# donahowe/TheaterGen

Hardware: AMD Instinct MI355X
Metric: 512px 50-step char images/sec (node), CMIGBench 4-turn story (higher is better)
Workload: dtype bf16; 1 GPU; SD-1.5 512x512, 4-turn story x 2 characters = 8 char images per step per GPU, 50 DDIM steps, CFG 7.5, IP-Adapter 77+4 tokens scale 0.4, bf16, random-init weights; plan=sd15, char_batch=8, cfg_batch=16, streams=1, ddim_steps=50, parallelism=dialogue-sharded x1 (RCCL broadcast + all_gather only)

## Files before the change

include/theatergen_hip.h:

```cpp
#ifndef THEATERGEN_HIP_H
#define THEATERGEN_HIP_H

#include <stdint.h>

#ifdef __cplusplus
extern "C" {
#endif

#define TG_BF16 0
#define TG_F16 1

#define TG_OK 0
#define TG_ERR_ARG (-1)
#define TG_ERR_LAUNCH (-2)
#define TG_ERR_UNSUPPORTED (-3)

#define TG_ACT_NONE 0
#define TG_ACT_SILU 1
#define TG_ACT_GELU 2
#define TG_ACT_QUICK_GELU 3

#define TG_ABI_VERSION 308
int tg_version(void);
const char* tg_last_error(void);
// ... 217 lines not shown
  int32_t dtype;
  const void* x; int64_t ldx;
  const void* wpk;
  const void* res; int64_t ldres;
  void* out; int64_t ldc;
  int64_t M;
  int32_t N, K;
  int32_t ln;
  float ln_eps;
  int32_t variant;
  const float* v640;
  const float* u640;
} tg_rc_linear_desc;
int tg_rc_linear(const tg_rc_linear_desc* d, void* stream);
int tg_rc_linear_dup(const tg_rc_linear_desc* d, int64_t c_dup_offset, void* stream);

typedef struct {
  int32_t dtype;
  const void* h; int64_t ldh;
  const void* wq;
  const void* kv;
  const void* wo;
  void* out; int64_t ldc;
  int64_t M;
  int32_t rows_per_batch;
  int32_t text_len, ip_tokens;
  float ln_eps;
  const float* ip_scale;
} tg_rc_xattn_desc;
int tg_rc_xattn(const tg_rc_xattn_desc* d, void* stream);
int tg_rc_kv_pack(int32_t dtype, int32_t batch, const void* k, const void* vt, int64_t ldt, int32_t text_len, const void* kip,
                  const void* vtip, int64_t ldi, int32_t ip_tokens, void* out, void* stream);

typedef struct {
  int32_t dtype;
  const void* h; int64_t ldh;
  const void* w1;
  const void* w2;
  const float* b2;
  const void* wpo;
  const void* res0; int64_t ldres;
  void* out; int64_t ldc;
  int64_t M;
  int32_t inner;
  float ln_eps;
  int32_t dbg;
} tg_rc_ff_desc;
int tg_rc_ff(const tg_rc_ff_desc* d, void* stream);

typedef struct {
  int32_t dtype;
  const void* x; int64_t ldx;
  const float* coef;
  const void* win;
  const void* wqkv;
  void* y; int64_t ldy;
  void* qk; int64_t ldqk;
  void* vt; int64_t ldt;
  int64_t M;
  int32_t rows_per_batch;
  float ln_eps;
  int32_t dbg;
} tg_rc_front_desc;
int tg_rc_front(const tg_rc_front_desc* d, void* stream);

typedef struct {
// ... 50 lines not shown
```

theatergen_amd/_lib.py:

```python
import ctypes as C
import os

HERE = os.path.dirname(os.path.abspath(__file__))
LIB_PATH = os.environ.get("THEATERGEN_HIP_LIB") or os.path.join(HERE, "lib", "libtheatergen_hip.so")

TG_BF16, TG_F16 = 0, 1
ABI_VERSION = 308
ACT_NONE, ACT_SILU, ACT_GELU, ACT_QUICK_GELU = 0, 1, 2, 3

i32, i64, f32, vp = C.c_int32, C.c_int64, C.c_float, C.c_void_p


class GemmDesc(C.Structure):
    _fields_ = [
        ("dtype", i32), ("mode", i32), ("a0", vp), ("a1", vp), ("c0", i32), ("c1", i32),
        ("batch", i32), ("in_h", i32), ("in_w", i32), ("out_h", i32), ("out_w", i32),
        ("stride", i32), ("upsample", i32), ("w", vp), ("M", i64), ("N", i64), ("K", i64),
        ("bias", vp), ("bvec", vp), ("ldbvec", i64), ("rows_per_batch", i64), ("res", vp), ("ldres", i64),
        ("act", i32), ("geglu", i32), ("out_scale", f32), ("out", vp), ("ldc", i64), ("n_split", i64),
        ("out_t", vp), ("ldt", i64), ("workspace", vp), ("workspace_bytes", i64),
        ("force_split_k", i32), ("force_tile", i32), ("a_rows_per_batch", i64), ("a_batch_stride", i64),
        ("pad_mode", i32), ("a_silu", i32), ("a_coef", vp), ("ln_u", vp), ("ln_v", vp), ("ln_eps", f32), ("ln_rows", vp),
        ("lda", i64), ("ldw", i64), ("out_gn_partials", vp), ("out_gn_groups", i32),
    ]


class AttnDesc(C.Structure):
    _fields_ = [
        ("dtype", i32), ("batch", i32), ("heads", i32), ("head_dim", i32), ("n_q", i32),
        ("q", vp), ("q_ld", i64), ("q_bs", i64),
        ("k0", vp), ("k0_ld", i64), ("k0_bs", i64), ("vt0", vp), ("vt0_ld", i64), ("vt0_bs", i64), ("len0", i32),
        ("k1", vp), ("k1_ld", i64), ("k1_bs", i64), ("vt1", vp), ("vt1_ld", i64), ("vt1_bs", i64), ("len1", i32),
        ("scale", f32), ("w1", f32), ("out", vp), ("out_ld", i64), ("out_bs", i64), ("causal", i32), ("w1_dev", vp),
        ("mask", vp), ("mask_bs", i64), ("mask_hs", i64), ("mask_qs", i64),
    ]


class AttnBwdDesc(C.Structure):
    _fields_ = [
        ("dtype", i32), ("batch", i32), ("heads", i32), ("head_dim", i32), ("n", i32),
        ("q", vp), ("k", vp), ("v", vp), ("dout", vp), ("ld", i64), ("bs", i64),
# ... 191 lines not shown
```

theatergen_amd/build.py:

```python
import hashlib
import os
import subprocess
import sys
from concurrent.futures import ThreadPoolExecutor

HERE = os.path.dirname(os.path.abspath(__file__))
CSRC = os.path.join(HERE, "csrc")
OBJ = os.path.join(CSRC, "_build")
LIBDIR = os.path.join(HERE, "lib")
LIB = os.path.join(LIBDIR, "libtheatergen_hip.so")
HEADER = os.path.join(os.path.dirname(HERE), "include", "theatergen_hip.h")
ARCH = "gfx950"
FLAGS = ["--offload-arch=" + ARCH, "-O3", "-std=c++17", "-fPIC",
         "-Wno-unused-result"]


EXTRA_FLAGS = {"tg_rowchain.hip": ["-mllvm", "-pragma-unroll-threshold=1000000"]}

BUILD_INFO = os.path.join(LIBDIR, "build_info.json")


def _write_build_info():
    import json

# ... 58 lines not shown
            f.write(r.stderr)
        with open(stamp, "w") as f:
            f.write(dg)

    if todo:
        with ThreadPoolExecutor(max_workers=min(8, len(todo))) as ex:
            list(ex.map(compile_one, todo))
    if todo or not os.path.exists(LIB):
        cmd = [hipcc, "--offload-arch=" + ARCH, "-shared", "-fPIC", "-o", LIB] + objs
        if verbose:
            print("[build]", " ".join(cmd), flush=True)
        r = subprocess.run(cmd, capture_output=True, text=True)
        if r.returncode != 0:
            raise RuntimeError(f"link failed:\n{r.stdout}\n{r.stderr}")
    if todo or not os.path.exists(BUILD_INFO):
        _write_build_info()
    if check_gate or os.environ.get("TG_BUILD_GATE") == "1":
        write_resources(check=True, verbose=verbose, report=False)
    return LIB


RESOURCES_JSON = os.path.join(os.path.dirname(HERE), "profiles", "r6_kernel_resources.json")
HOT_GATES = [
    ("attention_kernel<bf16,48,64,true,true,false,false>", 0, 128),
    ("attention_kernel<f16,48,64,true,true,false,false>", 0, 128),
    ("attention_kernel<", 0, 256),
    ("attention_wide_kernel<", 0, 256),
    ("gemm_glds_kernel<", 0, 256),
    ("conv_halo_kernel<", 0, 256),
    ("conv_slab_kernel<", 320, 256),
    ("bt_gemm_kernel<", 132, 256),
    ("rc_xattn_kernel<", 0, 256),
    ("rc_ff_kernel<", 0, 256),
    ("rc_front_kernel<", 0, 216),
    ("rc_linear_kernel<", 0, 256),
    ("skinny_gemm_kernel<", 0, 256),
    ("attn_bwd_kernel<4,2,", 0, 224),
    ("attn_bwd_kernel<", 0, 256),
    ("pp_gemm_kernel<bf16,2,", 0, 256),
    ("pp_gemm_kernel<f16,2,", 0, 256),
    ("pp_gemm_kernel<bf16,0,0>", 0, 256),
    ("pp_gemm_kernel<f16,0,0>", 0, 256),
    ("pp_gemm_kernel<", 256, 256),
    ("conv_in_mfma_kernel<", 0, 256),
    ("conv_out_mfma_kernel<", 0, 128),
    ("step_epilogue_kernel<", 0, 40),
]


def _pretty(sym):
    import re
    m = re.match(r"_ZN12_GLOBAL__N_1(\d+)", sym) or re.match(r"_Z(\d+)", sym)
    if not m:
        return sym
    n = int(m.group(1))
    base, rest = sym[m.end():m.end() + n], sym[m.end() + n:]
    if not rest.startswith("I"):
        return base
    args, i = [], 1
    while i < len(rest) and rest[i] != "E":
        if rest.startswith("DF16b", i):
            args.append("bf16"); i += 5
        elif rest.startswith("DF16_", i):
            args.append("f16"); i += 5
        elif rest.startswith("NS_", i):
            m = re.match(r"NS_(\d+)", rest[i:])
# ... 160 lines not shown
```

theatergen_amd/csrc/tg_rowchain.hip:

```cpp
#include "tg_common.h"

#include <type_traits>
#include <utility>

#ifdef TG_RC_DEV_BUILD
#define RC_DBG(bit) ((p.dbg & (bit)) != 0)
#define RC_DBG_ARG() (p.dbg >> 8)
#else
#define RC_DBG(bit) (false)
#define RC_DBG_ARG() (0)
#endif
#define RC_DBG_RT(bit) ((p.dbg & (bit)) != 0)

namespace {

struct RcLinearParams {
  const void* x;
  long ldx;
  const void* wpk;
  const void* res;
  long ldres;
  void* out;
  long ldc;
  long M;
// ... 1214 lines not shown
        f32x16 acc;
#pragma unroll
        for (int g = 0; g < 4; ++g) {
          const f32x4 v4 = *reinterpret_cast<const f32x4*>(vec + 4 * g);
#pragma unroll
          for (int e = 0; e < 4; ++e) acc[4 * g + e] = v4[e];
        }
        __builtin_amdgcn_sched_barrier(0);
#pragma unroll
        for (int x = 0; x < KS; ++x) {
          if (x + PD < KS) a[x + PD] = *reinterpret_cast<const V8*>(cb + (x + PD) * 1024);
          __builtin_amdgcn_sched_barrier(0);
          acc = mfma32(a[x], HB[x], acc);
          __builtin_amdgcn_sched_barrier(0);
        }
        if (uu == 0) quad_transpose(r8[0], r8[1], r8[2], r8[3]);
        float o[16];
#pragma unroll
        for (int r = 0; r < 16; ++r) o[r] = acc[r] + to_f32<T>(r8[2 * uu + (r >> 3)][r & 7]);
        pend[2 * uu] = pack8<T>(o);
        pend[2 * uu + 1] = pack8<T>(o + 8);
        if (uu == 1) quad_transpose(pend[0], pend[1], pend[2], pend[3]);
      }
    }
    {
      const long ch0 = 64 * 4 + 32 * hi;
#pragma unroll
      for (int i = 0; i < 4; ++i)
        if (mok[i]) *reinterpret_cast<V8*>(outp + mrow[i] * p.ldc + ch0 + 8 * qb) = pend[i];
    }
  }
}

template <typename T>
int launch_rc_ff(const tg_rc_ff_desc* d, const RcFfParams& p, hipStream_t st) {
  const size_t lds = 2 * 44 * 1024 + 2 * 20 * 1024;
  const long grid = (d->M + 127) / 128;
  if (d->wpo != nullptr) {
    auto k = rc_ff_kernel<T, true>;
    static const hipError_t attr = hipFuncSetAttribute(reinterpret_cast<const void*>(k), hipFuncAttributeMaxDynamicSharedMemorySize, (int)lds);
    (void)attr;
    hipLaunchKernelGGL(k, dim3((unsigned)grid), dim3(256), lds, st, p);
  } else {
    auto k = rc_ff_kernel<T, false>;
    static const hipError_t attr = hipFuncSetAttribute(reinterpret_cast<const void*>(k), hipFuncAttributeMaxDynamicSharedMemorySize, (int)lds);
    (void)attr;
    hipLaunchKernelGGL(k, dim3((unsigned)grid), dim3(256), lds, st, p);
  }
  TG_LAUNCH_CHECK();
  return TG_OK;
}

template <typename T, int KS, int NW, int NBUF, int PD>
int launch_rc_linear(const tg_rc_linear_desc* d, const RcLinearParams& p, hipStream_t st) {
  const size_t lds = (size_t)NBUF * (2 * KS + 1) * 1024;
  const long grid = (d->M + NW * 32 - 1) / (NW * 32);
  if (d->ln) {
    auto k = rc_linear_kernel<T, KS, NW, NBUF, true, PD>;
    static const hipError_t attr = hipFuncSetAttribute(reinterpret_cast<const void*>(k), hipFuncAttributeMaxDynamicSharedMemorySize, (int)lds);
    (void)attr;
    hipLaunchKernelGGL(k, dim3((unsigned)grid), dim3(NW * 64), lds, st, p);
  } else {
    auto k = rc_linear_kernel<T, KS, NW, NBUF, false, PD>;
    static const hipError_t attr = hipFuncSetAttribute(reinterpret_cast<const void*>(k), hipFuncAttributeMaxDynamicSharedMemorySize, (int)lds);
    (void)attr;
    hipLaunchKernelGGL(k, dim3((unsigned)grid), dim3(NW * 64), lds, st, p);
  }
  TG_LAUNCH_CHECK();
  return TG_OK;
}

template <typename T>
int dispatch_rc_linear(const tg_rc_linear_desc* d, const RcLinearParams& p, hipStream_t st) {
  switch (d->variant & 255) {
    case 1: return launch_rc_linear<T, 20, 8, 2, 4>(d, p, st);
    case 2: return launch_rc_linear<T, 20, 8, 3, 0>(d, p, st);
    case 3: return launch_rc_linear<T, 20, 8, 3, 4>(d, p, st);
    default: return launch_rc_linear<T, 20, 8, 2, 0>(d, p, st);
  }
}
// ... 44 lines not shown
  RcXattnParams p;
  p.h = d->h; p.ldh = d->ldh; p.wq = d->wq; p.kv = d->kv; p.wo = d->wo; p.out = d->out; p.ldc = d->ldc; p.M = d->M;
  p.rows_per_batch = d->rows_per_batch; p.ln_eps = d->ln_eps; p.ip_scale = d->ip_scale; p.dbg = d->text_len >> 8;
  hipStream_t st = reinterpret_cast<hipStream_t>(stream);
  if (d->dtype == TG_BF16) return dispatch_rc_xattn<bf16_t>(d, p, st);
  return dispatch_rc_xattn<f16_t>(d, p, st);
}

extern "C" int tg_rc_kv_pack(int32_t dtype, int32_t batch, const void* k, const void* vt, int64_t ldt, int32_t text_len, const void* kip,
                             const void* vtip, int64_t ldi, int32_t ip_tokens, void* out, void* stream) {
  TG_CHECK(dtype == TG_BF16 || dtype == TG_F16, TG_ERR_ARG, "tg_rc_kv_pack: dtype %d", dtype);
  TG_CHECK(batch > 0 && k && vt && out, TG_ERR_ARG, "tg_rc_kv_pack: null operand");
  TG_CHECK(text_len > 0 && text_len <= 80 && ip_tokens >= 0 && ip_tokens <= 16 && (ip_tokens == 0 || (kip && vtip)), TG_ERR_ARG,
           "tg_rc_kv_pack: %d text keys (<= 80), %d image keys (<= 16)", text_len, ip_tokens);
  hipStream_t st = reinterpret_cast<hipStream_t>(stream);
  const unsigned grid = (unsigned)batch * 8 * 24;
  if (dtype == TG_BF16)
    hipLaunchKernelGGL(rc_kv_pack_kernel<bf16_t>, dim3(grid), dim3(64), 0, st, (const bf16_t*)k, (const bf16_t*)vt, (long)ldt,
                       (const bf16_t*)kip, (const bf16_t*)vtip, (long)ldi, text_len, ip_tokens, (bf16_t*)out);
  else
    hipLaunchKernelGGL(rc_kv_pack_kernel<f16_t>, dim3(grid), dim3(64), 0, st, (const f16_t*)k, (const f16_t*)vt, (long)ldt,
                       (const f16_t*)kip, (const f16_t*)vtip, (long)ldi, text_len, ip_tokens, (f16_t*)out);
  TG_LAUNCH_CHECK();
  return TG_OK;
}

extern "C" int tg_rc_ff(const tg_rc_ff_desc* d, void* stream) {
  TG_CHECK(d != nullptr, TG_ERR_ARG, "tg_rc_ff: null descriptor");
  TG_CHECK(d->dtype == TG_BF16 || d->dtype == TG_F16, TG_ERR_ARG, "tg_rc_ff: dtype %d", d->dtype);
  TG_CHECK(d->h && d->w1 && d->w2 && d->b2 && d->out && d->M > 0, TG_ERR_ARG, "tg_rc_ff: null operand or M <= 0");
  TG_CHECK(d->inner >= 64 && d->inner % 64 == 0, TG_ERR_ARG, "tg_rc_ff: inner = %d must be a multiple of 64", d->inner);
  TG_CHECK(d->ldh >= 320 && d->ldh % 8 == 0 && d->ldc >= 320 && d->ldc % 8 == 0, TG_ERR_ARG, "tg_rc_ff: row pitches");
  TG_CHECK(!d->wpo || (d->res0 && d->ldres >= 320 && d->ldres % 8 == 0), TG_ERR_ARG, "tg_rc_ff: proj_out needs its residual");
  TG_CHECK(d->dbg == 0 || rc_dev_enabled(), TG_ERR_ARG, "tg_rc_ff: dbg = %d (dev switches need TG_RC_DEV=1)", d->dbg);
  RcFfParams p;
  p.h = d->h; p.ldh = d->ldh; p.w1 = d->w1; p.w2 = d->w2; p.b2 = d->b2; p.wpo = d->wpo; p.res0 = d->res0; p.ldres = d->ldres;
  p.out = d->out; p.ldc = d->ldc; p.M = d->M; p.n_slices = d->inner / 32; p.ln_eps = d->ln_eps; p.dbg = d->dbg;
  hipStream_t st = reinterpret_cast<hipStream_t>(stream);
  if (d->dtype == TG_BF16) return launch_rc_ff<bf16_t>(d, p, st);
  return launch_rc_ff<f16_t>(d, p, st);
}

extern "C" int tg_rc_front(const tg_rc_front_desc* d, void* stream) {
  TG_CHECK(d != nullptr, TG_ERR_ARG, "tg_rc_front: null descriptor");
  TG_CHECK(d->dtype == TG_BF16 || d->dtype == TG_F16, TG_ERR_ARG, "tg_rc_front: dtype %d", d->dtype);
  TG_CHECK(d->x && d->coef && d->win && d->wqkv && d->y && d->qk && d->vt && d->M > 0, TG_ERR_ARG, "tg_rc_front: null operand or M <= 0");
  TG_CHECK(d->rows_per_batch > 0 && d->rows_per_batch % 128 == 0 && d->M % d->rows_per_batch == 0, TG_ERR_ARG,
           "tg_rc_front: rows_per_batch = %d must be a multiple of 128 that divides M", d->rows_per_batch);
  TG_CHECK(d->ldx >= 320 && d->ldx % 8 == 0 && d->ldy >= 320 && d->ldy % 8 == 0 && d->ldqk >= 640 && d->ldqk % 8 == 0 && d->ldt >= d->rows_per_batch,
           TG_ERR_ARG, "tg_rc_front: row pitches");
  TG_CHECK(d->dbg == 0 || rc_dev_enabled(), TG_ERR_ARG, "tg_rc_front: dbg = %d (dev switches need TG_RC_DEV=1)", d->dbg);
  RcFrontParams p;
  p.x = d->x; p.ldx = d->ldx; p.coef = d->coef; p.win = d->win; p.wqkv = d->wqkv; p.y = d->y; p.ldy = d->ldy; p.qk = d->qk; p.ldqk = d->ldqk;
  p.vt = d->vt; p.ldt = d->ldt; p.M = d->M; p.rows_per_batch = d->rows_per_batch; p.ln_eps = d->ln_eps; p.dbg = d->dbg;
  hipStream_t st = reinterpret_cast<hipStream_t>(stream);
  if (d->dtype == TG_BF16) return launch_rc_front<bf16_t>(d, p, st);
  return launch_rc_front<f16_t>(d, p, st);
}
```

theatergen_amd/ops.py:

```python
import ctypes as C
import os

import torch

from . import _lib
from ._lib import ACT_GELU, ACT_NONE, ACT_QUICK_GELU, ACT_SILU, AttnDesc, GemmDesc

_workspaces = {}


def _dt(t):
    if t.dtype == torch.bfloat16:
        return _lib.TG_BF16
    if t.dtype == torch.float16:
        return _lib.TG_F16
    raise RuntimeError(f"theatergen_amd: unsupported activation dtype {t.dtype} (bf16 / fp16 only)")


def _stream():
    return torch.cuda.current_stream().cuda_stream


def _ptr(t):
    return None if t is None else t.data_ptr()
# ... 235 lines not shown
    d.kv, d.ip_scale = _ptr(kv), _ptr(ip_scale)
    d.out, d.ldc = _ptr(out), int(out.stride(0))
    d.M, d.C, d.head_dim, d.rows_per_batch, d.text_len, d.ip_tokens = int(M), int(Cc), int(head_dim), int(rows_per_batch), int(text_len), int(ip_tokens)
    L_ = text_len + ip_tokens
    flops = 2.0 * M * Cc * Cc + 4.0 * M * L_ * Cc
    tile = "128x128" if int(head_dim) == 64 else "128x160"
    _profiled(lambda: _lib.check(_lib.lib().tg_xq_attn(C.byref(d), _stream())), f"gemm_glds_kernel<plain+ln+xattn d{head_dim},{tile}>", M, Cc, Cc, flops,
              alg_bytes=2.0 * (2 * M * Cc + Cc * Cc) + 2.0 * (M // rows_per_batch) * 2 * L_ * Cc)
    return out


def rc_xattn(h, wq, kv, wo, rows_per_batch, ln_eps, ip_tokens, ip_scale=None, out=None, text_len=77):
    from ._lib import RcXattnDesc
    _need_cuda(h)
    M, Cc = h.shape
    assert Cc == 320 and h.stride(1) == 1
    if out is None:
        out = torch.empty(M, 320, dtype=h.dtype, device=h.device)
    d = RcXattnDesc()
    d.dtype = _dt(h)
    d.h, d.ldh = _ptr(h), int(h.stride(0))
    d.wq, d.kv, d.wo = _ptr(wq), _ptr(kv), _ptr(wo)
    d.out, d.ldc = _ptr(out), int(out.stride(0))
    d.M, d.rows_per_batch = int(M), int(rows_per_batch)
    d.text_len, d.ip_tokens = int(text_len), int(ip_tokens)
    d.ln_eps = float(ln_eps)
    d.ip_scale = _ptr(ip_scale)
    _profiled(lambda: _lib.check(_lib.lib().tg_rc_xattn(C.byref(d), _stream())), f"rc_xattn_kernel<77+{int(ip_tokens)}>",
              M, 320, 320, 4.0 * M * 320 * 320 + 4.0 * M * 320 * (int(text_len) + int(ip_tokens)), True,
              alg_bytes=2.0 * (3 * M * 320 + 2 * 320 * 320) + 2.0 * kv.numel())
    return out


def rc_ff(h, w1, w2, b2, inner, ln_eps, wpo=None, res0=None, out=None, dbg=0):
    from ._lib import RcFfDesc
    _need_cuda(h)
    M, Cc = h.shape
    assert Cc == 320 and h.stride(1) == 1
    if out is None:
        out = torch.empty(M, 320, dtype=h.dtype, device=h.device)
    d = RcFfDesc()
    d.dtype = _dt(h)
    d.h, d.ldh = _ptr(h), int(h.stride(0))
    d.w1, d.w2, d.b2, d.wpo = _ptr(w1), _ptr(w2), _ptr(b2), _ptr(wpo)
    d.res0, d.ldres = (_ptr(res0), int(res0.stride(0))) if res0 is not None else (None, 0)
    d.out, d.ldc = _ptr(out), int(out.stride(0))
    d.M, d.inner, d.ln_eps, d.dbg = int(M), int(inner), float(ln_eps), int(dbg)
    fl = 2.0 * M * 320 * (3 * int(inner)) + (2.0 * M * 320 * 320 if wpo is not None else 0.0)
    _profiled(lambda: _lib.check(_lib.lib().tg_rc_ff(C.byref(d), _stream())), "rc_ff_kernel<320>" + ("+proj_out" if wpo is not None else ""),
              M, 320, 3 * int(inner), fl, True,
              alg_bytes=2.0 * ((4 if wpo is not None else 3) * M * 320 + 3 * 320 * int(inner) + (320 * 320 if wpo is not None else 0)))
    return out


def rc_front(x, coef, win, wqkv, rows_per_batch, ln_eps, y=None, qk=None, vt=None, dbg=0):
    from ._lib import RcFrontDesc
    _need_cuda(x)
    M, Cc = x.shape
    assert Cc == 320 and x.stride(1) == 1 and coef.dtype == torch.float32
    B = M // rows_per_batch
    ldt = (rows_per_batch + 7) // 8 * 8
    if y is None:
        y = torch.empty(M, 320, dtype=x.dtype, device=x.device)
    if qk is None:
        qk = torch.empty(M, 640, dtype=x.dtype, device=x.device)
    if vt is None:
        vt = torch.empty(B, 320, ldt, dtype=x.dtype, device=x.device)
    d = RcFrontDesc()
    d.dtype = _dt(x)
    d.x, d.ldx, d.coef, d.win, d.wqkv = _ptr(x), int(x.stride(0)), _ptr(coef), _ptr(win), _ptr(wqkv)
    d.y, d.ldy, d.qk, d.ldqk, d.vt, d.ldt = _ptr(y), int(y.stride(0)), _ptr(qk), int(qk.stride(0)), _ptr(vt), int(vt.stride(1))
    d.M, d.rows_per_batch, d.ln_eps, d.dbg = int(M), int(rows_per_batch), float(ln_eps), int(dbg)
    fl = 2.0 * M * 320 * (320 + 960)
    _profiled(lambda: _lib.check(_lib.lib().tg_rc_front(C.byref(d), _stream())), "rc_front_kernel<320>", M, 960, 320, fl, False,
              alg_bytes=2.0 * (5 * M * 320 + 4 * 320 * 320))
    return y, qk, vt, int(vt.stride(1))


def skinny_gemm(x, wpk, N, *, ln=None, bias=None, act=ACT_NONE, res=None, out=None, segs=None, rows_per_batch=None):
    from ._lib import SkinnyDesc
    _need_cuda(x)
    M, K = x.shape
# ... 688 lines not shown
```

theatergen_amd/rowchain.py:

```python
import math
import os

import torch

from . import ops
from .weights_pack import rc_pack, rc_pack_tiles

ENABLED = os.environ.get("TG_RC", "1") != "0"
MODE = int(os.environ.get("TG_RC_MODE", "15"))
MIN_ROWS = int(os.environ.get("TG_RC_MIN_ROWS", "8192"))
MIN_ROWS_CHAIN = int(os.environ.get("TG_RC_MIN_ROWS_CHAIN", "32768"))
TRACE = os.environ.get("TG_RC_TRACE") == "1"


def trace(*a):
    if TRACE:
        print("[tg_rc]", *a, flush=True)

HEADS, DH, C = 8, 40, 320


def _q_slot_channels():
    out = torch.empty(C, dtype=torch.long)
    for n in range(C):
        c, hi, i, j = n // 64, (n // 32) & 1, (n // 8) & 3, n & 7
        s = 4 * c + i
        m, w5 = s // 5, s % 5
        if w5 == 0:
            head, d = 2 * m, 8 * hi + j
        elif w5 == 1:
            head, d = 2 * m, 16 + 8 * hi + j
        elif w5 == 2:
            head, d = (2 * m, 32 + j) if hi == 0 else (2 * m + 1, j)
        elif w5 == 3:
            head, d = 2 * m + 1, 8 + 8 * hi + j
        else:
            head, d = 2 * m + 1, 24 + 8 * hi + j
        out[n] = head * DH + d
    assert sorted(out.tolist()) == list(range(C))
    return out


# ... 72 lines not shown

def pack_ff(w1, b1, gamma, beta, w2, b2):
    from .weights_pack import _rc_maps
    inner = w2.shape[1]
    assert w1.shape == (2 * inner, C) and w2.shape == (C, inner) and inner % 32 == 0
    dev, dt = w1.device, w1.dtype
    g32, be32 = gamma.detach().float(), beta.detach().float()
    w1f = w1.detach().float()
    w1g = (w1f * g32[None, :]).to(dt)
    v1 = w1f @ be32 + (b1.detach().float() if b1 is not None else 0.0)
    pi, kap = _rc_maps(C)
    kap = kap.to(dev)
    rowoff = _ff_row_of().to(dev)
    ns = inner // 32
    hid = 32 * torch.arange(ns, device=dev)[:, None] + rowoff[None, :]
    rows_a, rows_g = hid, inner + hid
    rows = torch.stack([rows_a, rows_g], dim=1)
    frag = w1g[rows[:, :, None, None, :, None], kap[None, None, :, :, None, :]].contiguous()
    fb = frag.reshape(ns, -1).view(torch.uint8)
    page = torch.zeros(ns, 256, dtype=torch.float32, device=dev)
    acc_ch = (16 * torch.arange(2, device=dev)[:, None] + torch.arange(16, device=dev)[None, :]).reshape(-1)
    page[:, :32] = v1[(32 * torch.arange(ns, device=dev)[:, None] + acc_ch[None, :])]
    page[:, 32:64] = v1[inner + (32 * torch.arange(ns, device=dev)[:, None] + acc_ch[None, :])]
    s1 = torch.cat([fb, page.view(torch.uint8)], dim=1).reshape(-1)
    s1 = torch.cat([s1, torch.zeros(3 * 1024, dtype=torch.uint8, device=dev)])
    out_rows = (64 * torch.arange(C // 64)[:, None, None] + pi[None]).reshape(-1, 32).to(dev)
    kcol = (32 * torch.arange(ns, device=dev)[:, None, None, None] + 16 * torch.arange(2, device=dev)[None, None, :, None]
            + 8 * torch.arange(2, device=dev)[None, :, None, None] + torch.arange(8, device=dev)[None, None, None, :])
    w2d = w2.detach()
    f2 = w2d[out_rows[None, :, None, None, :, None], kcol[:, None, :, :, None, :]].contiguous()
    s2 = f2.reshape(-1).view(torch.uint8)
    bb2 = (b2.detach().float() if b2 is not None else torch.zeros(C, device=dev)).contiguous()
    return s1.contiguous(), s2.contiguous(), bb2
```

theatergen_amd/unet.py:

```python
from types import SimpleNamespace

import os

import torch
import torch.nn as nn

from . import ops
from . import rowchain
from .attention_processor import (tensor_version, Attention, AttnProcessor, CNAttnProcessor, IPAttnProcessor, _cached, front_eligible, fused_cross_block,
                                  ln_weight, pair_output, self_attention_from_qkv)
from .config import UNetConfig
from .weights_pack import pack_conv1x1, pack_conv3x3, pack_conv3x3_up2, pack_geglu, pack_ln_linear, rc_pack_tiles


class DeviceSchedule:

    def __init__(self, table, index):
        self.table, self.index = table, index


class _Act:
    __slots__ = ("t", "b", "h", "w", "c", "gn")

    def __init__(self, t, b, h, w, c, gn=None):
# ... 131 lines not shown

    def run(self, x: _Act):
        if _UP_FOLD and ops.conv_up2_eligible(x.t.dtype, x.b, x.h, x.w, x.c, self.conv.out_channels):
            wf = self._p.get("w_up2", [self.conv.weight], lambda: pack_conv3x3_up2(self.conv.weight.detach()))
            out = ops.conv_up2(x.t, wf, x.b, x.h, x.w, x.c, bias=self.conv.bias)
            return _Act(out, x.b, 2 * x.h, 2 * x.w, x.c)
        w = self._p.get("w", [self.conv.weight], lambda: pack_conv3x3(self.conv.weight.detach()))
        out = ops.conv3x3(x.t, w, x.b, x.h, x.w, x.c, upsample=True, bias=self.conv.bias)
        return _Act(out, x.b, 2 * x.h, 2 * x.w, x.c)


class GEGLU(nn.Module):
    def __init__(self, dim_in, dim_out):
        super().__init__()
        self.proj = nn.Linear(dim_in, dim_out * 2)


class FeedForward(nn.Module):

    def __init__(self, dim, mult=4):
        super().__init__()
        inner = dim * mult
        self.net = nn.ModuleList([GEGLU(dim, inner), nn.Dropout(0.0), nn.Linear(inner, dim)])
        self._p = _Packed()

    def run_fused(self, x2d, norm, tail=None):
        proj, lin2 = self.net[0].proj, self.net[2]
        M, K = x2d.shape
        inner = lin2.weight.shape[1]
        if (not rowchain.ENABLED or not (rowchain.MODE & 4) or K != 320 or lin2.weight.shape[0] != 320 or inner % 64 or M < rowchain.MIN_ROWS_CHAIN
                or x2d.stride(0) != K or proj.weight.shape[0] != 2 * inner):
            return None
        ts = [proj.weight, proj.bias, norm.weight, norm.bias, lin2.weight] + ([lin2.bias] if lin2.bias is not None else [])
        s1, s2, b2 = self._p.get("rc_ff", ts, lambda: rowchain.pack_ff(proj.weight, proj.bias, norm.weight, norm.bias, lin2.weight, lin2.bias))
        wpo = res0 = None
        if tail is not None:
            w_out, b_out, res0 = tail
            wpo = self._p.get("rc_po", [w_out] + ([b_out] if b_out is not None else []),
                              lambda: rc_pack_tiles(w_out.detach(), b_out.detach().float() if b_out is not None else None))
        return ops.rc_ff(x2d, s1, s2, b2, inner, norm.eps, wpo=wpo, res0=res0)

    def _hidden(self, M, inner, like):
        if _FF_PAD and inner % 512 == 0:
            return torch.empty((M, inner + 64), dtype=like.dtype, device=like.device)[:, :inner]
        return torch.empty((M, inner), dtype=like.dtype, device=like.device)

    def _w2(self):
        w2 = self.net[2].weight
        inner = w2.shape[1]
        if not (_FF_PAD and inner % 512 == 0):
            return w2

        def build():
            wp = torch.zeros((w2.shape[0], inner + 64), dtype=w2.dtype, device=w2.device)
            wp[:, :inner] = w2.detach()
            return wp
        return self._p.get("w2pad", [w2], build)[:, :inner]

    def run(self, x2d, residual, ln=None):
        proj = self.net[0].proj
        M, K = x2d.shape
        inner = proj.weight.shape[0] // 2
        if ln is not None:
            norm, rows = ln

            def build():
                wp, bp = pack_geglu(proj.weight.detach(), proj.bias.detach())
                return pack_ln_linear(wp, bp, norm.weight, norm.bias)
            wl, ul, vl = self._p.get("geglu_ln", [proj.weight, proj.bias, norm.weight, norm.bias], build)
            g = ops.gemm(x2d, wl, M, wl.shape[0], K, geglu=True, ln=(ul, vl, norm.eps, rows), out=self._hidden(M, inner, x2d))
        elif M > 64 and inner % 32 == 0:
            wp, bp = self._p.get("geglu", [proj.weight, proj.bias], lambda: pack_geglu(proj.weight.detach(), proj.bias.detach()))
            g = ops.gemm(x2d, wp, M, wp.shape[0], K, bias=bp, geglu=True, out=self._hidden(M, inner, x2d))
# ... 538 lines not shown
```

Baseline: 9.816 char_images/s.

## Add two-wave-per-SIMD fused feed-forward kernel with repacked weights, enable by default

Result: faster. 9.921 char_images/s, median of 6 (+1.1%).

```diff
diff --git a/include/theatergen_hip.h b/include/theatergen_hip.h
--- a/include/theatergen_hip.h
+++ b/include/theatergen_hip.h
@@ -273,6 +273,7 @@
 int tg_rc_kv_pack(int32_t dtype, int32_t batch, const void* k, const void* vt, int64_t ldt, int32_t text_len, const void* kip,
                   const void* vtip, int64_t ldi, int32_t ip_tokens, void* out, void* stream);
 
+#define TG_RC_FF_TWO_WAVE 0x10000
 typedef struct {
   int32_t dtype;
   const void* h; int64_t ldh;
diff --git a/theatergen_amd/_lib.py b/theatergen_amd/_lib.py
--- a/theatergen_amd/_lib.py
+++ b/theatergen_amd/_lib.py
@@ -7,6 +7,7 @@
 TG_BF16, TG_F16 = 0, 1
 ABI_VERSION = 308
 ACT_NONE, ACT_SILU, ACT_GELU, ACT_QUICK_GELU = 0, 1, 2, 3
+RC_FF_TWO_WAVE = 0x10000
 
 i32, i64, f32, vp = C.c_int32, C.c_int64, C.c_float, C.c_void_p
 
diff --git a/theatergen_amd/build.py b/theatergen_amd/build.py
--- a/theatergen_amd/build.py
+++ b/theatergen_amd/build.py
@@ -114,6 +114,7 @@
     ("bt_gemm_kernel<", 132, 256),
     ("rc_xattn_kernel<", 0, 256),
     ("rc_ff_kernel<", 0, 256),
+    ("rc_ff2_kernel<", 0, 256),
     ("rc_front_kernel<", 0, 216),
     ("rc_linear_kernel<", 0, 256),
     ("skinny_gemm_kernel<", 0, 256),
diff --git a/theatergen_amd/csrc/tg_rowchain.hip b/theatergen_amd/csrc/tg_rowchain.hip
--- a/theatergen_amd/csrc/tg_rowchain.hip
+++ b/theatergen_amd/csrc/tg_rowchain.hip
@@ -1270,20 +1270,301 @@
   }
 }
 
+template <typename T, bool PROJ>
+__global__ __launch_bounds__(512) __attribute__((amdgpu_waves_per_eu(2, 2))) void rc_ff2_kernel(RcFfParams p) {
+  typedef typename Vec<T>::v8 V8;
+  constexpr int KS = 10, NW = 8;
+  constexpr int W1B = 41 * 1024, W1SLOT = 44 * 1024, W2B = 20 * 1024;
+  constexpr int W2OFF = 2 * W1SLOT;
+  constexpr int TBW = 21 * 1024, SLOT = 24 * 1024;
+  extern __shared__ __attribute__((aligned(16))) char smem[];
+
+  const int tid = threadIdx.x;
+  const int lane = tid & 63;
+  const int wave = __builtin_amdgcn_readfirstlane(tid >> 6);
+  const int n = lane & 15, g = lane >> 4;
+  const int lbid = rc_block_id((int)blockIdx.x, (int)gridDim.x);
+  const long tok = ((long)lbid * NW + wave) * 16 + n;
+  const bool ok = tok < p.M;
+  const long row = ok ? tok : p.M - 1;
+  const int NS = p.n_slices;
+  const char* w1g = reinterpret_cast<const char*>(p.w1) + lane * 16 + wave * 1024;
+  const char* w2g = reinterpret_cast<const char*>(p.w2) + lane * 16 + wave * 1024;
+  auto issue_w1 = [&](int j) __attribute__((always_inline)) {
+    const char* s0 = w1g + (long)j * W1B;
+    char* dst = smem + (j & 1) * W1SLOT + wave * 1024;
+#pragma unroll
+    for (int q = 0; q < 6; ++q)
+      if (q < 5 || wave < 4)
+        __builtin_amdgcn_global_load_lds((const __attribute__((address_space(1))) void*)(s0 + q * NW * 1024),
+                                         (__attribute__((address_space(3))) void*)(dst + q * NW * 1024), 16, 0, 0);
+  };
+  auto issue_w2 = [&](int j) __attribute__((always_inline)) {
+    const char* s0 = w2g + (long)j * W2B;
+    char* dst = smem + W2OFF + (j & 1) * W2B + wave * 1024;
+#pragma unroll
+    for (int q = 0; q < 3; ++q)
+      if (q < 2 || wave < 4)
+        __builtin_amdgcn_global_load_lds((const __attribute__((address_space(1))) void*)(s0 + q * NW * 1024),
+                                         (__attribute__((address_space(3))) void*)(dst + q * NW * 1024), 16, 0, 0);
+  };
+  issue_w1(0);
+
+  V8 HN[KS];
+  {
+    V8 H[KS];
+    const T* xp = reinterpret_cast<const T*>(p.h) + row * p.ldh + 8 * g;
+#pragma unroll
+    for (int s = 0; s < KS; ++s) H[s] = *reinterpret_cast<const V8*>(xp + 32 * s);
+    float sum = 0.f;
+#pragma unroll
+    for (int s = 0; s < KS; ++s)
+#pragma unroll
+      for (int e = 0; e < 8; ++e) sum += to_f32<T>(H[s][e]);
+    sum += __shfl_xor(sum, 16, 64);
+    sum += __shfl_xor(sum, 32, 64);
+    const float mean = sum * (1.0f / 320.0f);
+    float c2 = 0.f;
+#pragma unroll
+    for (int s = 0; s < KS; ++s) {
+      asm volatile("" : "+v"(H[s]));
+#pragma unroll
+      for (int e = 0; e < 8; ++e) { const float d = to_f32<T>(H[s][e]) - mean; c2 = __builtin_fmaf(d, d, c2); }
+    }
+    c2 += __shfl_xor(c2, 16, 64);
+    c2 += __shfl_xor(c2, 32, 64);
+    const float rstd = __builtin_amdgcn_rsqf(c2 * (1.0f / 320.0f) + p.ln_eps);
+    const float nm = -mean * rstd;
+#pragma unroll
+    for (int s = 0; s < KS; ++s) {
+      asm volatile("" : "+v"(H[s]));
+      float f[8];
+#pragma unroll
+      for (int e = 0; e < 8; ++e) f[e] = __builtin_fmaf(to_f32<T>(H[s][e]), rstd, nm);
+      HN[s] = pack8<T>(f);
+    }
+  }
+  f32x4 out[20];
+#pragma unroll
+  for (int t = 0; t < 20; ++t) out[t] = *reinterpret_cast<const f32x4*>(p.b2 + 32 * (t >> 1) + 8 * g + 4 * (t & 1));
+
+  f32x4 acc_a[2][2], acc_g[2][2];
+  V8 hid[2];
+#pragma unroll
+  for (int q = 0; q < 2; ++q)
+#pragma unroll
+    for (int e = 0; e < 8; ++e) hid[q][e] = from_f32<T>(0.f);
+
+  auto iteration = [&](int j, auto par_c, auto f1_c, auto gg_c, auto f2_c) __attribute__((always_inline)) {
+    constexpr int PAR = decltype(par_c)::value;
+    constexpr bool F1 = decltype(f1_c)::value, GG = decltype(gg_c)::value, F2 = decltype(f2_c)::value;
+    asm volatile("s_waitcnt vmcnt(0)" ::: "memory");
+    __builtin_amdgcn_s_barrier();
+    if (j + 1 < NS) issue_w1(j + 1);
+    if (j >= 1 && j - 1 < NS) issue_w2(j - 1);
+    constexpr int LA = 9;
+    const unsigned lbase = (unsigned)reinterpret_cast<size_t>((__attribute__((address_space(3))) char*)smem);
+    const unsigned a1 = lbase + PAR * W1SLOT + lane * 16, a2 = lbase + W2OFF + PAR * W2B + lane * 16;
+    V8 fr[60];
+    auto rd = [&](auto xc) __attribute__((always_inline)) {
+      constexpr int x = decltype(xc)::value;
+      constexpr int k = x / 3, w = x % 3;
+      if constexpr (w == 0) { if constexpr (F1) lds_read16<k * 1024>(fr[x], a1); }
+      else if constexpr (w == 1) { if constexpr (F1) lds_read16<(20 + k) * 1024>(fr[x], a1); }
+      else { if constexpr (F2) lds_read16<k * 1024>(fr[x], a2); }
+    };
+    if constexpr (F1) {
+      const unsigned ap = lbase + PAR * W1SLOT + 40 * 1024 + g * 16;
+      lds_read16<0>(acc_a[PAR][0], ap);
+      lds_read16<64>(acc_a[PAR][1], ap);
+      lds_read16<128>(acc_g[PAR][0], ap);
+      lds_read16<192>(acc_g[PAR][1], ap);
+    }
+    static_for<LA>([&](auto xc) __attribute__((always_inline)) { rd(xc); });
+    float ge_z = 0.f, ge_t = 0.f, ge_p = 0.f;
+    float hv[8];
+    auto geglu_micro = [&](int mstep) __attribute__((always_inline)) {
+      const int e = mstep >> 2, part = mstep & 3;
+      const float a = acc_a[PAR ^ 1][e >> 2][e & 3], gt = acc_g[PAR ^ 1][e >> 2][e & 3];
+      if (part == 0) {
+        ge_z = __builtin_amdgcn_fmed3f(gt * 0.70710678118654752440f, -3.0f, 3.0f);
+        ge_t = ge_z * ge_z;
+      } else if (part == 1) {
+        float q = __builtin_fmaf(-4.0553346e-07f, ge_t, 1.7159753e-05f);
+        q = __builtin_fmaf(q, ge_t, -3.1459445e-04f);
+        q = __builtin_fmaf(q, ge_t, 3.3187051e-03f);
+        ge_p = __builtin_fmaf(q, ge_t, -2.2685785e-02f);
+      } else if (part == 2) {
+        float q = __builtin_fmaf(ge_p, ge_t, 1.0771781e-01f);
+        q = __builtin_fmaf(q, ge_t, -3.7323141e-01f);
+        q = __builtin_fmaf(q, ge_t, 1.1278958f);
+        ge_p = q * ge_z;
+      } else {
+        hv[e] = a * gt * __builtin_fmaf(0.5f, ge_p, 0.5f);
+        if (e == 7) hid[PAR ^ 1] = pack8<T>(hv);
+      }
+    };
+    __builtin_amdgcn_sched_barrier(0);
+    static_for<60>([&](auto xc) __attribute__((always_inline)) {
+      constexpr int x = decltype(xc)::value;
+      constexpr int k = x / 3, w = x % 3;
+      constexpr bool act = (w == 2) ? F2 : F1;
+      if constexpr (F1 && F2) {
+        if constexpr (w == 0) {
+          if constexpr (x + LA < 60) rd(std::integral_constant<int, (x + LA < 60 ? x + LA : 59)>{});
+          if constexpr (x + LA + 1 < 60) rd(std::integral_constant<int, (x + LA + 1 < 60 ? x + LA + 1 : 59)>{});
+          if constexpr (x + LA + 2 < 60) rd(std::integral_constant<int, (x + LA + 2 < 60 ? x + LA + 2 : 59)>{});
+        }
+      } else {
+        if constexpr (x + LA < 60) rd(std::integral_constant<int, (x + LA < 60 ? x + LA : 59)>{});
+      }
+      __builtin_amdgcn_sched_barrier(0);
+      if constexpr (act) {
+        constexpr int hi_x = x + LA < 60 ? x + LA : 59;
+        constexpr int n_f1 = ((hi_x / 3) * 2 + (hi_x % 3 >= 1 ? 2 : 1)) - ((x / 3) * 2 + (x % 3 >= 1 ? 2 : 1));
+        constexpr int n_f2 = (hi_x + 1) / 3 - (x + 1) / 3;
+        constexpr int younger = (F1 ? n_f1 : 0) + (F2 ? n_f2 : 0);
+        if constexpr (F1 && F2) {
+          if constexpr (w == 0) {
+            constexpr int hi3 = x + 2 + LA < 60 ? x + 2 + LA : 59;
+            lds_wait3<(hi3 - (x + 2) > 15 ? 15 : hi3 - (x + 2))>(fr[x], fr[x + 1], fr[x + 2]);
+          }
+        } else {
+          lds_wait<(younger > 15 ? 15 : younger)>(fr[x]);
+        }
+        if constexpr (F1 && x == 0) asm volatile("" : "+v"(acc_a[PAR][0]), "+v"(acc_a[PAR][1]), "+v"(acc_g[PAR][0]), "+v"(acc_g[PAR][1]));
+        if constexpr (w == 0) acc_a[PAR][k & 1] = mfma16(fr[x], HN[k >> 1], acc_a[PAR][k & 1]);
+        else if constexpr (w == 1) acc_g[PAR][k & 1] = mfma16(fr[x], HN[k >> 1], acc_g[PAR][k & 1]);
+        else out[k] = mfma16(fr[x], hid[PAR], out[k]);
+      }
+      __builtin_amdgcn_sched_barrier(0);
+      if constexpr (GG) {
+        constexpr int m0 = 32 * x / 60, m1 = 32 * (x + 1) / 60;
+        if constexpr (m1 > m0) {
+          geglu_micro(m0);
+          __builtin_amdgcn_sched_barrier(0);
+        }
+      }
+    });
+    if constexpr (GG) asm volatile("" :: "v"(hid[PAR ^ 1]));
+  };
+  using C0 = std::integral_constant<int, 0>;
+  using C1 = std::integral_constant<int, 1>;
+  using Tt = std::true_type;
+  using Ff = std::false_type;
+  iteration(0, C0{}, Tt{}, Ff{}, Ff{});
+  iteration(1, C1{}, Tt{}, Tt{}, Ff{});
+  for (int j = 2; j < NS; j += 2) {
+    iteration(j, C0{}, Tt{}, Tt{}, Tt{});
+    iteration(j + 1, C1{}, Tt{}, Tt{}, Tt{});
+  }
+  iteration(NS, C0{}, Ff{}, Tt{}, Tt{});
+  iteration(NS + 1, C1{}, Ff{}, Ff{}, Tt{});
+
+  {
+    const T* hb = reinterpret_cast<const T*>(p.h);
+    asm volatile("" : "+s"(hb));
+    const T* xp = hb + row * p.ldh + 8 * g;
+#pragma unroll
+    for (int s = 0; s < KS; ++s) {
+      const V8 hr = gld<V8>(xp + 32 * s);
+#pragma unroll
+      for (int e = 0; e < 8; ++e) out[2 * s + (e >> 2)][e & 3] += to_f32<T>(hr[e]);
+    }
+  }
+  auto pack_rows = [&](int s) __attribute__((always_inline)) {
+    float f[8];
+#pragma unroll
+    for (int e = 0; e < 8; ++e) f[e] = out[2 * s + (e >> 2)][e & 3];
+    return pack8<T>(f);
+  };
+
+  T* outp = reinterpret_cast<T*>(p.out);
+  if constexpr (!PROJ) {
+    asm volatile("" : "+s"(outp));
+    T* op = outp + row * p.ldc + 8 * g;
+#pragma unroll
+    for (int s = 0; s < KS; ++s) {
+      const V8 pc = pack_rows(s);
+      if (ok) gst<V8>(op + 32 * s, pc);
+    }
+  } else {
+    V8 HB[KS];
+#pragma unroll
+    for (int s = 0; s < KS; ++s) HB[s] = pack_rows(s);
+    const char* wpg = reinterpret_cast<const char*>(p.wpo) + lane * 16 + wave * 1024;
+    auto issue_po = [&](int st) __attribute__((always_inline)) {
+      if (st >= 10) return;
+      const char* s0 = wpg + (long)st * TBW;
+      char* dst = smem + (st % 3) * SLOT + wave * 1024;
+#pragma unroll
+      for (int q = 0; q < 3; ++q)
+        __builtin_amdgcn_global_load_lds((const __attribute__((address_space(1))) void*)(s0 + q * NW * 1024),
+                                         (__attribute__((address_space(3))) void*)(dst + q * NW * 1024), 16, 0, 0);
+    };
+    __builtin_amdgcn_s_barrier();
+    issue_po(0);
+    issue_po(1);
+    const T* rp = reinterpret_cast<const T*>(p.res0);
+    asm volatile("" : "+s"(rp), "+s"(outp));
+    rp += row * p.ldres + 8 * g;
+    T* op = outp + row * p.ldc + 8 * g;
+    const unsigned pbase = (unsigned)reinterpret_cast<size_t>((__attribute__((address_space(3))) char*)smem) + lane * 16;
+#pragma unroll
+    for (int st = 0; st < 10; ++st) {
+      if (st == 0) asm volatile("s_waitcnt vmcnt(3)" ::: "memory");
+      else if (st == 9) asm volatile("s_waitcnt vmcnt(1)" ::: "memory");
+      else asm volatile("s_waitcnt vmcnt(4)" ::: "memory");
+      __builtin_amdgcn_s_barrier();
+      V8 r8;
+      asm volatile("global_load_dwordx4 %0, %1, off" : "=v"(r8) : "v"(rp + 32 * st) : "memory");
+      issue_po(st + 2);
+      const unsigned cb = pbase + (st % 3) * SLOT;
+      constexpr int PD = 8;
+      V8 a[20];
+      f32x4 acc[2];
+      lds_read16<20 * 1024>(acc[0], cb - lane * 16 + g * 16);
+      lds_read16<20 * 1024 + 64>(acc[1], cb - lane * 16 + g * 16);
+      static_for<PD>([&](auto xc) __attribute__((always_inline)) { constexpr int x = decltype(xc)::value; lds_read16<x * 1024>(a[x], cb); });
+      __builtin_amdgcn_sched_barrier(0);
+      static_for<20>([&](auto xc) __attribute__((always_inline)) {
+        constexpr int x = decltype(xc)::value;
+        if constexpr (x + PD < 20) lds_read16<(x + PD < 20 ? x + PD : 0) * 1024>(a[x + PD < 20 ? x + PD : 0], cb);
+        lds_wait<(x + PD < 20 ? PD : 19 - x)>(a[x]);
+        if constexpr (x == 0) asm volatile("" : "+v"(acc[0]), "+v"(acc[1]));
+        __builtin_amdgcn_sched_barrier(0);
+        acc[x & 1] = mfma16(a[x], HB[x >> 1], acc[x & 1]);
+        __builtin_amdgcn_sched_barrier(0);
+      });
+      if (st + 2 < 10) asm volatile("s_waitcnt vmcnt(3)" : "+v"(r8));
+      else asm volatile("s_waitcnt vmcnt(0)" : "+v"(r8));
+      float o[8];
+#pragma unroll
+      for (int e = 0; e < 8; ++e) o[e] = acc[e >> 2][e & 3] + to_f32<T>(r8[e]);
+      const V8 pc = pack8<T>(o);
+      if (ok) gst<V8>(op + 32 * st, pc);
+    }
+  }
+}
+
+template <void (*K)(RcFfParams)>
+void launch_rc_ff_kernel(long grid, int threads, size_t lds, hipStream_t st, const RcFfParams& p) {
+  static const hipError_t attr = hipFuncSetAttribute(reinterpret_cast<const void*>(K), hipFuncAttributeMaxDynamicSharedMemorySize, (int)lds);
+  (void)attr;
+  hipLaunchKernelGGL(K, dim3((unsigned)grid), dim3(threads), lds, st, p);
+}
+
 template <typename T>
 int launch_rc_ff(const tg_rc_ff_desc* d, const RcFfParams& p, hipStream_t st) {
   const size_t lds = 2 * 44 * 1024 + 2 * 20 * 1024;
   const long grid = (d->M + 127) / 128;
+  const bool two = (d->dbg & TG_RC_FF_TWO_WAVE) != 0;
   if (d->wpo != nullptr) {
-    auto k = rc_ff_kernel<T, true>;
-    static const hipError_t attr = hipFuncSetAttribute(reinterpret_cast<const void*>(k), hipFuncAttributeMaxDynamicSharedMemorySize, (int)lds);
-    (void)attr;
-    hipLaunchKernelGGL(k, dim3((unsigned)grid), dim3(256), lds, st, p);
+    if (two) launch_rc_ff_kernel<rc_ff2_kernel<T, true>>(grid, 512, lds, st, p);
+    else launch_rc_ff_kernel<rc_ff_kernel<T, true>>(grid, 256, lds, st, p);
   } else {
-    auto k = rc_ff_kernel<T, false>;
-    static const hipError_t attr = hipFuncSetAttribute(reinterpret_cast<const void*>(k), hipFuncAttributeMaxDynamicSharedMemorySize, (int)lds);
-    (void)attr;
-    hipLaunchKernelGGL(k, dim3((unsigned)grid), dim3(256), lds, st, p);
+    if (two) launch_rc_ff_kernel<rc_ff2_kernel<T, false>>(grid, 512, lds, st, p);
+    else launch_rc_ff_kernel<rc_ff_kernel<T, false>>(grid, 256, lds, st, p);
   }
   TG_LAUNCH_CHECK();
   return TG_OK;
@@ -1394,10 +1675,10 @@
   TG_CHECK(d->inner >= 64 && d->inner % 64 == 0, TG_ERR_ARG, "tg_rc_ff: inner = %d must be a multiple of 64", d->inner);
   TG_CHECK(d->ldh >= 320 && d->ldh % 8 == 0 && d->ldc >= 320 && d->ldc % 8 == 0, TG_ERR_ARG, "tg_rc_ff: row pitches");
   TG_CHECK(!d->wpo || (d->res0 && d->ldres >= 320 && d->ldres % 8 == 0), TG_ERR_ARG, "tg_rc_ff: proj_out needs its residual");
-  TG_CHECK(d->dbg == 0 || rc_dev_enabled(), TG_ERR_ARG, "tg_rc_ff: dbg = %d (dev switches need TG_RC_DEV=1)", d->dbg);
+  TG_CHECK((d->dbg & ~TG_RC_FF_TWO_WAVE) == 0 || rc_dev_enabled(), TG_ERR_ARG, "tg_rc_ff: dbg = %d (dev switches need TG_RC_DEV=1)", d->dbg);
   RcFfParams p;
   p.h = d->h; p.ldh = d->ldh; p.w1 = d->w1; p.w2 = d->w2; p.b2 = d->b2; p.wpo = d->wpo; p.res0 = d->res0; p.ldres = d->ldres;
-  p.out = d->out; p.ldc = d->ldc; p.M = d->M; p.n_slices = d->inner / 32; p.ln_eps = d->ln_eps; p.dbg = d->dbg;
+  p.out = d->out; p.ldc = d->ldc; p.M = d->M; p.n_slices = d->inner / 32; p.ln_eps = d->ln_eps; p.dbg = d->dbg & ~TG_RC_FF_TWO_WAVE;
   hipStream_t st = reinterpret_cast<hipStream_t>(stream);
   if (d->dtype == TG_BF16) return launch_rc_ff<bf16_t>(d, p, st);
   return launch_rc_ff<f16_t>(d, p, st);
diff --git a/theatergen_amd/ops.py b/theatergen_amd/ops.py
--- a/theatergen_amd/ops.py
+++ b/theatergen_amd/ops.py
@@ -291,7 +291,7 @@
     return out
 
 
-def rc_ff(h, w1, w2, b2, inner, ln_eps, wpo=None, res0=None, out=None, dbg=0):
+def rc_ff(h, w1, w2, b2, inner, ln_eps, wpo=None, res0=None, out=None, dbg=0, two_wave=False):
     from ._lib import RcFfDesc
     _need_cuda(h)
     M, Cc = h.shape
@@ -304,9 +304,9 @@
     d.w1, d.w2, d.b2, d.wpo = _ptr(w1), _ptr(w2), _ptr(b2), _ptr(wpo)
     d.res0, d.ldres = (_ptr(res0), int(res0.stride(0))) if res0 is not None else (None, 0)
     d.out, d.ldc = _ptr(out), int(out.stride(0))
-    d.M, d.inner, d.ln_eps, d.dbg = int(M), int(inner), float(ln_eps), int(dbg)
+    d.M, d.inner, d.ln_eps, d.dbg = int(M), int(inner), float(ln_eps), int(dbg) | (_lib.RC_FF_TWO_WAVE if two_wave else 0)
     fl = 2.0 * M * 320 * (3 * int(inner)) + (2.0 * M * 320 * 320 if wpo is not None else 0.0)
-    _profiled(lambda: _lib.check(_lib.lib().tg_rc_ff(C.byref(d), _stream())), "rc_ff_kernel<320>" + ("+proj_out" if wpo is not None else ""),
+    _profiled(lambda: _lib.check(_lib.lib().tg_rc_ff(C.byref(d), _stream())), ("rc_ff2_kernel<320>" if two_wave else "rc_ff_kernel<320>") + ("+proj_out" if wpo is not None else ""),
               M, 320, 3 * int(inner), fl, True,
               alg_bytes=2.0 * ((4 if wpo is not None else 3) * M * 320 + 3 * 320 * int(inner) + (320 * 320 if wpo is not None else 0)))
     return out
diff --git a/theatergen_amd/rowchain.py b/theatergen_amd/rowchain.py
--- a/theatergen_amd/rowchain.py
+++ b/theatergen_amd/rowchain.py
@@ -7,7 +7,8 @@
 from .weights_pack import rc_pack, rc_pack_tiles
 
 ENABLED = os.environ.get("TG_RC", "1") != "0"
-MODE = int(os.environ.get("TG_RC_MODE", "15"))
+MODE = int(os.environ.get("TG_RC_MODE", "47"))
+FF_TWO_WAVE = ops._lib.RC_FF_TWO_WAVE
 MIN_ROWS = int(os.environ.get("TG_RC_MIN_ROWS", "8192"))
 MIN_ROWS_CHAIN = int(os.environ.get("TG_RC_MIN_ROWS_CHAIN", "32768"))
 TRACE = os.environ.get("TG_RC_TRACE") == "1"
@@ -146,3 +147,51 @@
     s2 = f2.reshape(-1).view(torch.uint8)
     bb2 = (b2.detach().float() if b2 is not None else torch.zeros(C, device=dev)).contiguous()
     return s1.contiguous(), s2.contiguous(), bb2
+
+
+def _ff2_out_row():
+    r = torch.arange(16)
+    return torch.stack([8 * (r >> 2) + 4 * u + (r & 3) for u in range(2)])
+
+
+def pack_ff2(w1, b1, gamma, beta, w2, b2):
+    inner = w2.shape[1]
+    assert w1.shape == (2 * inner, C) and w2.shape == (C, inner) and inner % 32 == 0
+    dev, dt = w1.device, w1.dtype
+    ar = lambda k: torch.arange(k, device=dev)
+    w1f = w1.detach().float()
+    w1g = (w1f * gamma.detach().float()[None, :]).to(dt)
+    v1 = w1f @ beta.detach().float() + (b1.detach().float() if b1 is not None else 0.0)
+    ns = inner // 32
+    rows = (inner * ar(2)[None, :, None, None, None, None, None] + 32 * ar(ns)[:, None, None, None, None, None, None]
+            + 16 * ar(2)[None, None, None, :, None, None, None] + ar(16)[None, None, None, None, None, :, None])
+    cols = 32 * ar(10)[None, None, :, None, None, None, None] + 8 * ar(4)[None, None, None, None, :, None, None] + ar(8)
+    fb = w1g[rows, cols].contiguous().reshape(ns, -1).view(torch.uint8)
+    page = torch.zeros(ns, 256, dtype=torch.float32, device=dev)
+    page[:, :32] = v1[:inner].reshape(ns, 32)
+    page[:, 32:64] = v1[inner:].reshape(ns, 32)
+    s1 = torch.cat([fb, page.view(torch.uint8)], dim=1).reshape(-1)
+    s1 = torch.cat([s1, torch.zeros(3 * 1024, dtype=torch.uint8, device=dev)])
+    orow = _ff2_out_row().to(dev)
+    out_rows = (32 * ar(10)[:, None, None] + orow[None]).reshape(20, 16)
+    e = ar(8)
+    kcol = (32 * ar(ns)[:, None, None] + 4 * ar(4)[None, :, None] + (16 * (e >> 2) + (e & 3))[None, None, :])
+    f2 = w2.detach()[out_rows[None, :, None, :, None], kcol[:, None, :, None, :]].contiguous()
+    s2 = f2.reshape(-1).view(torch.uint8)
+    bb2 = (b2.detach().float() if b2 is not None else torch.zeros(C, device=dev)).contiguous()
+    return s1.contiguous(), s2.contiguous(), bb2
+
+
+def pack_po2(w, b=None):
+    assert w.shape == (C, C)
+    dev = w.device
+    ar = lambda k: torch.arange(k, device=dev)
+    orow = _ff2_out_row().to(dev)
+    rows = 32 * ar(10)[:, None, None, None, None, None] + orow[None, None, :, None, :, None]
+    cols = 32 * ar(10)[None, :, None, None, None, None] + 8 * ar(4)[None, None, None, :, None, None] + ar(8)
+    fb = w.detach()[rows, cols].contiguous().reshape(10, -1).view(torch.uint8)
+    page = torch.zeros(10, 256, dtype=torch.float32, device=dev)
+    if b is not None:
+        page[:, :32] = b.detach().float()[(32 * ar(10)[:, None, None] + orow[None]).reshape(10, 32)]
+    out = torch.cat([fb, page.view(torch.uint8)], dim=1).contiguous().reshape(-1)
+    return torch.cat([out, torch.zeros(3 * 1024, dtype=torch.uint8, device=dev)])
diff --git a/theatergen_amd/unet.py b/theatergen_amd/unet.py
--- a/theatergen_amd/unet.py
+++ b/theatergen_amd/unet.py
@@ -187,13 +187,16 @@
                 or x2d.stride(0) != K or proj.weight.shape[0] != 2 * inner):
             return None
         ts = [proj.weight, proj.bias, norm.weight, norm.bias, lin2.weight] + ([lin2.bias] if lin2.bias is not None else [])
-        s1, s2, b2 = self._p.get("rc_ff", ts, lambda: rowchain.pack_ff(proj.weight, proj.bias, norm.weight, norm.bias, lin2.weight, lin2.bias))
+        two = bool(rowchain.MODE & 32)
+        pack = rowchain.pack_ff2 if two else rowchain.pack_ff
+        s1, s2, b2 = self._p.get("rc_ff2" if two else "rc_ff", ts, lambda: pack(proj.weight, proj.bias, norm.weight, norm.bias, lin2.weight, lin2.bias))
         wpo = res0 = None
         if tail is not None:
             w_out, b_out, res0 = tail
-            wpo = self._p.get("rc_po", [w_out] + ([b_out] if b_out is not None else []),
-                              lambda: rc_pack_tiles(w_out.detach(), b_out.detach().float() if b_out is not None else None))
-        return ops.rc_ff(x2d, s1, s2, b2, inner, norm.eps, wpo=wpo, res0=res0)
+            pack_po = rowchain.pack_po2 if two else rc_pack_tiles
+            wpo = self._p.get("rc_po2" if two else "rc_po", [w_out] + ([b_out] if b_out is not None else []),
+                              lambda: pack_po(w_out.detach(), b_out.detach().float() if b_out is not None else None))
+        return ops.rc_ff(x2d, s1, s2, b2, inner, norm.eps, wpo=wpo, res0=res0, two_wave=two)
 
     def _hidden(self, M, inner, like):
         if _FF_PAD and inner % 512 == 0:
```
